# gebegebegebe/onnx-transformer

Hardware: AMD Instinct MI355X
Metric: decoded tokens/sec IWSLT14 de-en int8 greedy (batch 32 over 1 GPU, 71 steps) (higher is better)
Workload: dtype int8; 1 GPU; cfg2: greedy decode, src<=64 padded to 72, max_len=72, 32 sentences length-sorted over 1 rank(s); global_batch=32, per_gpu_batch=32, seq_len=72, parallelism=sentence-shard x1

## Files before the change

onnx-transformer_amd/csrc/qtx_common.h:

```cpp
#pragma once
#include <hip/hip_runtime.h>
#include <stdint.h>

#include <type_traits>

#define QTX_WAVE 64

typedef int v4i __attribute__((ext_vector_type(4)));
typedef float v4f __attribute__((ext_vector_type(4)));
typedef int v16i __attribute__((ext_vector_type(16)));

#ifdef QTX_STAMPS
static __device__ unsigned long long* qtx_stamp_buf;
#define QTX_STAMP_SETTER(unit)                                                            \
  extern "C" int qtx_debug_set_stamps_##unit(void* buf) {                                 \
    return (int)hipMemcpyToSymbol(HIP_SYMBOL(qtx_stamp_buf), &buf, sizeof(buf));          \
  }
#define QTX_STAMP(slot)                                                                 \
  do {                                                                                    \
    if (threadIdx.x == 0 && qtx_stamp_buf)                                                \
      qtx_stamp_buf[(blockIdx.y * gridDim.x + blockIdx.x) * 16 + (slot)] =                \
          __builtin_amdgcn_s_memtime();                                                   \
  } while (0)
#define QTX_NOW() ((long long)__builtin_amdgcn_s_memtime())
// ... 38 lines not shown
  v = fmaxf(v, dpp<0x141>(v));
  v = fmaxf(v, dpp<0x140>(v));
  return fmaxf(fmaxf(lane_f(v, 0), lane_f(v, 16)), fmaxf(lane_f(v, 32), lane_f(v, 48)));
}

template <int R>
__device__ __forceinline__ void wave_sum_n(float (&v)[R]) {
#pragma unroll
  for (int j = 0; j < R; ++j) v[j] = v[j] + dpp<0xB1>(v[j]);
#pragma unroll
  for (int j = 0; j < R; ++j) v[j] = v[j] + dpp<0x4E>(v[j]);
#pragma unroll
  for (int j = 0; j < R; ++j) v[j] = v[j] + dpp<0x141>(v[j]);
#pragma unroll
  for (int j = 0; j < R; ++j) v[j] = v[j] + dpp<0x140>(v[j]);
#pragma unroll
  for (int j = 0; j < R; ++j) v[j] = (lane_f(v[j], 0) + lane_f(v[j], 16)) + (lane_f(v[j], 32) + lane_f(v[j], 48));
}
template <int R>
__device__ __forceinline__ void wave_max_n(float (&v)[R]) {
#pragma unroll
  for (int j = 0; j < R; ++j) v[j] = fmaxf(v[j], dpp<0xB1>(v[j]));
#pragma unroll
  for (int j = 0; j < R; ++j) v[j] = fmaxf(v[j], dpp<0x4E>(v[j]));
#pragma unroll
  for (int j = 0; j < R; ++j) v[j] = fmaxf(v[j], dpp<0x141>(v[j]));
#pragma unroll
  for (int j = 0; j < R; ++j) v[j] = fmaxf(v[j], dpp<0x140>(v[j]));
#pragma unroll
  for (int j = 0; j < R; ++j)
    v[j] = fmaxf(fmaxf(lane_f(v[j], 0), lane_f(v[j], 16)), fmaxf(lane_f(v[j], 32), lane_f(v[j], 48)));
}

__device__ __forceinline__ float row16_sum(float v) {
  v = v + dpp<0xB1>(v);
  v = v + dpp<0x4E>(v);
  v = v + dpp<0x141>(v);
  return v + dpp<0x140>(v);
}
__device__ __forceinline__ float row16_max(float v) {
  v = fmaxf(v, dpp<0xB1>(v));
  v = fmaxf(v, dpp<0x4E>(v));
  v = fmaxf(v, dpp<0x141>(v));
  return fmaxf(v, dpp<0x140>(v));
}

__device__ __forceinline__ int wave_min_i32(int v) {
  auto d = [](int x, auto ctrl) {
    return __builtin_amdgcn_update_dpp(0x7fffffff, x, decltype(ctrl)::value, 0xF, 0xF, false);
  };
  v = min(v, d(v, std::integral_constant<int, 0xB1>{}));
  v = min(v, d(v, std::integral_constant<int, 0x4E>{}));
  v = min(v, d(v, std::integral_constant<int, 0x141>{}));
  v = min(v, d(v, std::integral_constant<int, 0x140>{}));
  return min(min(__builtin_amdgcn_readlane(v, 0), __builtin_amdgcn_readlane(v, 16)),
             min(__builtin_amdgcn_readlane(v, 32), __builtin_amdgcn_readlane(v, 48)));
}
template <int CTRL>
__device__ __forceinline__ int dpp_i32(int v) {
  return __builtin_amdgcn_update_dpp(0, v, CTRL, 0xF, 0xF, true);
}
__device__ __forceinline__ int row16_min_i32(int v) {
  v = min(v, dpp_i32<0xB1>(v));
  v = min(v, dpp_i32<0x4E>(v));
  v = min(v, dpp_i32<0x141>(v));
  return min(v, dpp_i32<0x140>(v));
// ... 128 lines not shown
__device__ __forceinline__ bool divisor_ok(float b) {
  const uint32_t m = __float_as_uint(b) & 0x7fffffffu;
  return m - 0x30800001u < 0x4e800000u - 0x30800001u;
}

__device__ __forceinline__ float div_const(float a, float b) {
  const float y = 1.0f / b;
  if (__builtin_expect(__ballot(!div_ok(a)) == 0ull, 1)) return div_cr(a, b, y);
  return a / b;
}
template <int R>
__device__ __forceinline__ void div_const_n(float (&a)[R], float b) {
  const float y = 1.0f / b;
  bool bad = false;
#pragma unroll
  for (int j = 0; j < R; ++j) bad |= !div_ok(a[j]);
  if (__builtin_expect(__ballot(bad) == 0ull, 1)) {
#pragma unroll
    for (int j = 0; j < R; ++j) a[j] = div_cr(a[j], b, y);
  } else {
#pragma unroll
    for (int j = 0; j < R; ++j) a[j] = a[j] / b;
  }
}

__device__ __forceinline__ float div127(float c) {
  return fmaf(c, 0x1.020408p-7f, c * 0x1.020408p-35f);
}

__device__ __forceinline__ float quant_scale(float absmax, float qmax) {
  return div_const(fmaxf(absmax, 1e-5f), qmax);
}
__device__ __forceinline__ int quant_val(float x, float s) { return (int)rintf(x / s); }
__device__ __forceinline__ float scale127(float a) {
  const bool big = a >= 0x1p60f;
  const float q = div_cr(big ? a * 0x1p-64f : a, 127.0f, 1.0f / 127.0f);
  return a == __builtin_inff() ? a : (big ? q * 0x1p64f : q);
}
__device__ __forceinline__ float rcp_cr(float s) {
  const float y0 = __builtin_amdgcn_rcpf(s);
  const float y = fmaf(fmaf(-s, y0, 1.0f), y0, y0);
  return s == __builtin_inff() ? 0.0f : y;
}

__device__ __forceinline__ uint32_t pack4_i8(int a, int b, int c, int d) {
  return (uint32_t)(a & 0xff) | ((uint32_t)(b & 0xff) << 8) | ((uint32_t)(c & 0xff) << 16) |
         ((uint32_t)(d & 0xff) << 24);
}

__host__ __device__ __forceinline__ long kp_off(long r, long k, long K) {
  return (((r >> 1) * (K >> 6) + (k >> 6)) << 7) + ((r & 1) << 6) + (k & 63);
}

template <class T>
__device__ __forceinline__ const T& ld_at(const T* base, unsigned byte_off) {
  return *reinterpret_cast<const T*>(reinterpret_cast<const char*>(base) + byte_off);
}
template <class T>
__device__ __forceinline__ void st_at(T* base, unsigned byte_off, const T& v) {
  *reinterpret_cast<T*>(reinterpret_cast<char*>(base) + byte_off) = v;
}

__device__ __forceinline__ float rint_biased(float q) { return q + 12582912.0f; }
__device__ __forceinline__ uint32_t pack4_biased(float t0, float t1, float t2, float t3) {
  const uint32_t p01 = __builtin_amdgcn_perm(__float_as_uint(t1), __float_as_uint(t0), 0x0c0c0400u);
  const uint32_t p23 = __builtin_amdgcn_perm(__float_as_uint(t3), __float_as_uint(t2), 0x0c0c0400u);
// ... 7 lines not shown
}
template <bool RELU>
__device__ __forceinline__ uint32_t pack4_codes(float q0, float q1, float q2, float q3) {
  if constexpr (RELU) return pack4_relu_u8(q0, q1, q2, q3);
  else return pack4_biased(rint_biased(q0), rint_biased(q1), rint_biased(q2), rint_biased(q3));
}

template <int N>
__device__ __forceinline__ void quant_pack(const float* x, float s, uint32_t* out) {
  static_assert(N % 4 == 0, "groups of 4");
  constexpr float BIAS = 12582912.0f;
  const float inv = __builtin_amdgcn_rcpf(s);
  float t[N];
  float dm = 0.0f;
#pragma unroll
  for (int i = 0; i < N; ++i) {
    const float r = x[i] * inv;
    t[i] = r + BIAS;
    dm = fmaxf(dm, fabsf(r - (t[i] - BIAS)));
  }
  if (__builtin_expect(__ballot(dm > 0.5f - 0x1p-13f) != 0ull, 0)) {
#pragma unroll
    for (int i = 0; i < N; ++i) t[i] = x[i] / s + BIAS;
  }
#pragma unroll
  for (int i = 0; i < N / 4; ++i) out[i] = pack4_biased(t[4 * i], t[4 * i + 1], t[4 * i + 2], t[4 * i + 3]);
}
__device__ __forceinline__ int quant_one(float x, float s) {
  float r = x * __builtin_amdgcn_rcpf(s);
  const bool near = fabsf((r - floorf(r)) - 0.5f) < 0x1p-13f;
  if (__builtin_expect(__ballot(near) != 0ull, 0)) r = x / s;
  return (int)rintf(r);
}

template <class PSF, class VF>
__device__ __forceinline__ float pv_dec_chains(int Sk, PSF&& ps, VF&& v) {
  float c[4] = {0.0f, 0.0f, 0.0f, 0.0f};
  for (int g = 0; g < Sk; g += 16)
#pragma unroll
    for (int e = 0; e < 4; ++e)
#pragma unroll
      for (int q = 0; q < 4; ++q) {
        const int j = g + 4 * q + e;
        if (j < Sk) c[q] = fmaf(ps(j), v(j), c[q]);
      }
  return (c[0] + c[1]) + (c[2] + c[3]);
}

__device__ __forceinline__ unsigned abs_bits(float x) { return __float_as_uint(fabsf(x)); }

template <int R>
__device__ __forceinline__ void ln_rows512(float (&v)[R][2][4], const float (&ga)[2][4],
                                           const float (&gb)[2][4]) {
  float mean[R], den[R];
#pragma unroll
  for (int j = 0; j < R; ++j) {
    float s = v[j][0][0];
#pragma unroll
    for (int c = 0; c < 2; ++c)
#pragma unroll
      for (int e = 0; e < 4; ++e)
        if (c | e) s = s + v[j][c][e];
    mean[j] = s;
  }
  wave_sum_n<R>(mean);
#pragma unroll
// ... 50 lines not shown
#pragma unroll
      for (int c = 0; c < 2; ++c)
#pragma unroll
        for (int e = 0; e < 4; ++e) v[j][c][e] = div_cr(v[j][c][e], den[j], y) + gb[c][e];
    }
  } else {
#pragma unroll
    for (int j = 0; j < R; ++j)
#pragma unroll
      for (int c = 0; c < 2; ++c)
#pragma unroll
        for (int e = 0; e < 4; ++e) v[j][c][e] = v[j][c][e] / den[j] + gb[c][e];
  }
}

__device__ __forceinline__ void ln_params512(const float* a, const float* b, int lane,
                                             float (&ga)[2][4], float (&gb)[2][4]) {
#pragma unroll
  for (int c = 0; c < 2; ++c) {
    const float4 ta = *reinterpret_cast<const float4*>(a + 4 * (lane + 64 * c));
    const float4 tb = *reinterpret_cast<const float4*>(b + 4 * (lane + 64 * c));
    ga[c][0] = ta.x; ga[c][1] = ta.y; ga[c][2] = ta.z; ga[c][3] = ta.w;
    gb[c][0] = tb.x; gb[c][1] = tb.y; gb[c][2] = tb.z; gb[c][3] = tb.w;
  }
}
template <int R>
__device__ __forceinline__ void ln_rows512(float (&v)[R][2][4], const float* a, const float* b,
                                           int lane) {
  float ga[2][4], gb[2][4];
  ln_params512(a, b, lane, ga, gb);
  ln_rows512<R>(v, ga, gb);
}

template <int R>
__device__ __forceinline__ void quant_rows512(const float (&v)[R][2][4], uint32_t (&q)[R][2],
                                              float (&sc)[R]) {
#pragma unroll
  for (int j = 0; j < R; ++j) {
    sc[j] = 0.0f;
#pragma unroll
    for (int c = 0; c < 2; ++c)
#pragma unroll
      for (int e = 0; e < 4; ++e) sc[j] = fmaxf(sc[j], fabsf(v[j][c][e]));
  }
  wave_max_n<R>(sc);
#pragma unroll
  for (int j = 0; j < R; ++j) sc[j] = fmaxf(sc[j], 1e-5f);
  div_const_n<R>(sc, 127.0f);
  constexpr float BIAS = 12582912.0f;
  float t[R][8];
  float dm = 0.0f;
#pragma unroll
  for (int j = 0; j < R; ++j) {
    const float inv = __builtin_amdgcn_rcpf(sc[j]);
#pragma unroll
    for (int i = 0; i < 8; ++i) {
      const float r = v[j][i >> 2][i & 3] * inv;
      t[j][i] = r + BIAS;
      dm = fmaxf(dm, fabsf(r - (t[j][i] - BIAS)));
    }
  }
  if (__builtin_expect(__ballot(dm > 0.5f - 0x1p-13f) != 0ull, 0)) {
#pragma unroll
    for (int j = 0; j < R; ++j)
#pragma unroll
      for (int i = 0; i < 8; ++i) t[j][i] = v[j][i >> 2][i & 3] / sc[j] + BIAS;
  }
#pragma unroll
  for (int j = 0; j < R; ++j) {
    q[j][0] = pack4_biased(t[j][0], t[j][1], t[j][2], t[j][3]);
    q[j][1] = pack4_biased(t[j][4], t[j][5], t[j][6], t[j][7]);
  }
}

}
```

onnx-transformer_amd/csrc/qtx_decode.hip:

```cpp
#include <cstdlib>

#include "qtx_common.h"
#include "qtx_kernels.h"
#include "qtx_knobs.h"

QTX_STAMP_SETTER(decode)

namespace qtx {

__device__ __forceinline__ uint4 unpack_i4(uint2 h) {
  auto sext = [](uint32_t v) { return v | ((v & 0x08080808u) * 0x1Eu); };
  const uint32_t lo0 = sext(h.x & 0x0F0F0F0Fu), hi0 = sext((h.x >> 4) & 0x0F0F0F0Fu);
  const uint32_t lo1 = sext(h.y & 0x0F0F0F0Fu), hi1 = sext((h.y >> 4) & 0x0F0F0F0Fu);
  uint4 o;
  o.x = __builtin_amdgcn_perm(hi0, lo0, 0x05010400u);
  o.y = __builtin_amdgcn_perm(hi0, lo0, 0x07030602u);
  o.z = __builtin_amdgcn_perm(hi1, lo1, 0x05010400u);
  o.w = __builtin_amdgcn_perm(hi1, lo1, 0x07030602u);
  return o;
}

struct KaLead { uint64_t w[7]; };
#define QTX_KA_PARAMS uint64_t ka0, uint64_t ka1, uint64_t ka2, uint64_t ka3, uint64_t ka4, \
                      uint64_t ka5, uint64_t ka6
// ... 84 lines not shown
    }
    issue_rest();
    if (tid < BM) sas[tid] = (tid < RB && m0 + tid < g.M) ? g.sa[m0 + tid] : 0.0f;
#pragma unroll
    for (int j = 0; j < NLD; ++j) {
      const int idx = tid + 256 * j, r = idx / CPR;
      if (TOT % 256 == 0 || idx < TOT)
        *reinterpret_cast<uint4*>(As + r * LDA + 16 * (idx % CPR)) =
            (m0 + r < g.M) ? v[j] : make_uint4(0, 0, 0, 0);
    }
  } else if constexpr (AMODE == A_LN) {
    float v[RPW][2][4];
#pragma unroll
    for (int j = 0; j < RPW; ++j) {
      const int m = min(m0 + wave + 4 * j, g.M - 1);
#pragma unroll
      for (int c = 0; c < 2; ++c) {
        const float4 t = ld_at(reinterpret_cast<const float4*>(g.X), 4u * (unsigned)(m * (int)g.ldx + 4 * (lane + 64 * c)));
        v[j][c][0] = t.x; v[j][c][1] = t.y; v[j][c][2] = t.z; v[j][c][3] = t.w;
      }
    }
    float ga[2][4], gb[2][4];
    ln_params512(g.ln_a, g.ln_b, lane, ga, gb);
    issue_rest();
    uint32_t q[RPW][2];
    float sc[RPW];
#if defined(QTX_ABL) && (QTX_ABL & 2)
#pragma unroll
    for (int j = 0; j < RPW; ++j) {
      q[j][0] = __float_as_uint(v[j][0][0]); q[j][1] = __float_as_uint(v[j][1][0]); sc[j] = v[j][0][1];
    }
#else
    ln_rows512<RPW>(v, ga, gb);
    quant_rows512<RPW>(v, q, sc);
#endif
#pragma unroll
    for (int j = 0; j < RPW; ++j) {
      const int r = wave + 4 * j;
      const bool ok = m0 + r < g.M;
      uint32_t* dst = reinterpret_cast<uint32_t*>(As + r * LDA);
      dst[lane] = ok ? q[j][0] : 0u;
      dst[lane + 64] = ok ? q[j][1] : 0u;
      if (lane == 0) sas[r] = ok ? sc[j] : 0.0f;
    }
  } else {
    constexpr bool OWN = AMODE == A_F32R;
    constexpr int NC = K / 256, RBT = RPW < 4 ? RPW : 4;
#pragma unroll
    for (int j0 = 0; j0 < RPW; j0 += RBT) {
      float4 t[RBT][NC];
      float pm[RBT][2];
#pragma unroll
      for (int jb = 0; jb < RBT; ++jb) {
        const int m = min(m0 + wave + 4 * (j0 + jb), g.M - 1);
#pragma unroll
        for (int c = 0; c < NC; ++c)
          t[jb][c] = ld_at(reinterpret_cast<const float4*>(g.X), 4u * (unsigned)(m * (int)g.ldx + 4 * (lane + 64 * c)));
        if constexpr (!OWN)
#pragma unroll
          for (int u = 0; u < 2; ++u)
            pm[jb][u] = ld_at(g.pmax_in, 4u * (unsigned)(min(lane + 64 * u, g.pmax_n - 1) * g.M + m));
      }
      if (j0 == 0) issue_rest();
#pragma unroll
      for (int jb = 0; jb < RBT; ++jb) {
        const int r = wave + 4 * (j0 + jb);
        const bool ok = m0 + r < g.M;
        float lm;
        if constexpr (OWN) {
          lm = 0.0f;
#pragma unroll
          for (int c = 0; c < NC; ++c)
            lm = fmaxf(lm, fmaxf(fmaxf(fabsf(t[jb][c].x), fabsf(t[jb][c].y)),
                                 fmaxf(fabsf(t[jb][c].z), fabsf(t[jb][c].w))));
        } else {
          lm = fmaxf(pm[jb][0], pm[jb][1]);
        }
        const float sc = quant_scale(wave_max(lm), 127.0f);
        uint32_t* dst = reinterpret_cast<uint32_t*>(As + r * LDA);
        float tf[4 * NC];
#pragma unroll
        for (int c = 0; c < NC; ++c) {
          tf[4 * c] = t[jb][c].x; tf[4 * c + 1] = t[jb][c].y;
          tf[4 * c + 2] = t[jb][c].z; tf[4 * c + 3] = t[jb][c].w;
        }
        uint32_t qd[NC];
#if defined(QTX_ABL) && (QTX_ABL & 8)
#pragma unroll
        for (int c = 0; c < NC; ++c) qd[c] = __float_as_uint(tf[4 * c] * sc);
#else
        quant_pack<4 * NC>(tf, sc, qd);
#endif
#pragma unroll
        for (int c = 0; c < NC; ++c) dst[lane + 64 * c] = ok ? qd[c] : 0u;
        if (lane == 0) sas[r] = ok ? sc : 0.0f;
      }
    }
  }
}

template <int MF, int RB, int K, int WBITS, int AMODE, int FLAGS>
__global__ __launch_bounds__(256) void k_skinny(QTX_KA_PARAMS, SkTail kt) {
  const SkinnyArgs g = sk_args<AMODE>(QTX_KA_VALS, kt);
  constexpr int BM = 16 * MF;
  static_assert(RB % 4 == 0 && RB <= BM, "rows per block");
  constexpr int KW = K / 4;
  constexpr int NS = KW / 64;
  constexpr int LDA = K + 16;
  __shared__ __attribute__((aligned(16))) uint8_t As[BM * LDA];
  __shared__ float sas[BM];
  __shared__ v4i red[4][MF][64];
// ... 72 lines not shown
  const int e = wave;
#pragma unroll
  for (int i = 0; i < MF; ++i) {
    {
      int sum = 0;
#pragma unroll
      for (int w = 0; w < 4; ++w) sum += reinterpret_cast<const int*>(&red[w][i][lane])[e];
      const int r = 16 * i + 4 * fg + e, row = m0 + r;
      const bool ok = cok && r < RB && row < g.M;
      float y = ((float)sum * sas[r]) * swc + bc;
      if constexpr (relu) y = y > 0.0f ? y : 0.0f;
      if constexpr (resid) y = rv[i] + y;
      if (ok) st_at(g.out, 4u * (unsigned)(row * (int)g.ldo + col), y);
      if constexpr (rmax) {
        float am = ok ? fabsf(y) : 0.0f;
        am = fmaxf(am, dpp<0xB1>(am));
        am = fmaxf(am, dpp<0x4E>(am));
        am = fmaxf(am, dpp<0x141>(am));
        am = fmaxf(am, dpp<0x140>(am));
        if (fr == 0 && r < RB && row < g.M) g.pmax_out[(long)blockIdx.x * g.M + row] = am;
      }
    }
  }
  QTX_STAMP(3);
}

template <bool OWN>
__global__ __launch_bounds__(512) void k_skinny8_ffn2(QTX_KA_PARAMS, SkTail kt) {
  const SkinnyArgs g = sk_args<OWN ? A_F32R : A_F32Q>(QTX_KA_VALS, kt);
  constexpr int K = 2048, RB = 4, KW = K / 8, NS = KW / 64, LDA = K + 16;
  __shared__ __attribute__((aligned(16))) uint8_t As[16 * LDA];
  __shared__ float sas[16];
  __shared__ v4i red[8][64];
  __shared__ float hmax[8];
  const int tid = threadIdx.x, wave = tid >> 6, lane = tid & 63;
  const int fr = lane & 15, fg = lane >> 4;
  const int n0 = blockIdx.x * 16, m0 = blockIdx.y * RB;
  const int r = wave >> 1, half = wave & 1;
  const int m = min(m0 + r, g.M - 1);
  float4 t[4];
#pragma unroll
  for (int c = 0; c < 4; ++c)
    t[c] = ld_at(reinterpret_cast<const float4*>(g.X), 4u * (unsigned)(m * (int)g.ldx + 4 * (lane + 64 * (4 * half + c))));
  float pm[2] = {0.0f, 0.0f};
  if constexpr (!OWN)
#pragma unroll
    for (int u = 0; u < 2; ++u) pm[u] = ld_at(g.pmax_in, 4u * (unsigned)(min(lane + 64 * u, g.pmax_n - 1) * g.M + m));
  const int n = min(n0 + fr, g.N - 1);
  uint4 wf[NS];
#pragma unroll
  for (int s = 0; s < NS; ++s)
    wf[s] = ld_at(reinterpret_cast<const uint4*>(g.W), (unsigned)(n * (int)g.ldw + wave * KW + 64 * s + 16 * fg));
  const int col = n0 + fr, cc = min(col, g.N - 1);
  const bool cok = col < g.N;
  const float swc = ld_at(g.sw, 4u * cc);
  __builtin_amdgcn_sched_barrier(0);
  const float rv = ld_at(g.res, 4u * (unsigned)(min(m0 + fg, g.M - 1) * (int)g.ldr + cc));
  const float bc = ld_at(g.bias, 4u * cc);
  {
    const bool ok = m0 + r < g.M;
    float rmax;
    if constexpr (OWN) {
      float lm = 0.0f;
#pragma unroll
      for (int c = 0; c < 4; ++c)
        lm = fmaxf(lm, fmaxf(fmaxf(fabsf(t[c].x), fabsf(t[c].y)), fmaxf(fabsf(t[c].z), fabsf(t[c].w))));
      lm = wave_max(lm);
      if (lane == 0) hmax[wave] = lm;
      __syncthreads();
      rmax = fmaxf(hmax[2 * r], hmax[2 * r + 1]);
    } else {
      rmax = wave_max(fmaxf(pm[0], pm[1]));
    }
    const float sc = quant_scale(rmax, 127.0f);
    float tf[16];
#pragma unroll
    for (int c = 0; c < 4; ++c) {
      tf[4 * c] = t[c].x; tf[4 * c + 1] = t[c].y; tf[4 * c + 2] = t[c].z; tf[4 * c + 3] = t[c].w;
    }
    uint32_t qd[4];
    quant_pack<16>(tf, sc, qd);
    uint32_t* dst = reinterpret_cast<uint32_t*>(As + r * LDA);
#pragma unroll
    for (int c = 0; c < 4; ++c) dst[lane + 64 * (4 * half + c)] = ok ? qd[c] : 0u;
    if (lane == 0 && half == 0) sas[r] = ok ? sc : 0.0f;
  }
  __syncthreads();
  v4i acc = v4i{0, 0, 0, 0};
#pragma unroll
  for (int s = 0; s < NS; ++s) {
    const v4i afr = *reinterpret_cast<const v4i*>(As + fr * LDA + wave * KW + 64 * s + 16 * fg);
    acc = __builtin_amdgcn_mfma_i32_16x16x64_i8(afr, __builtin_bit_cast(v4i, wf[s]), acc, 0, 0, 0);
  }
  red[wave][lane] = acc;
  __syncthreads();
  if (wave != 0) return;
  {
    const int e = fg, src = fr;
    int sum = 0;
#pragma unroll
    for (int w = 0; w < 8; ++w) sum += reinterpret_cast<const int*>(&red[w][src])[e];
    const int row = m0 + e;
    const float y = ((float)sum * sas[e]) * swc + bc;
    if (cok && row < g.M) st_at(g.out, 4u * (unsigned)(row * (int)g.ldo + col), rv + y);
  }
}

// ... 234 lines not shown
constexpr int DEC_MAXK = 128;

template <bool KV_NEW> struct DaLead;
template <> struct DaLead<true> {
  uint64_t y; int ldy, kv_bs; uint64_t kc, vc, skc, svc; int host_step1, zero;
};
template <> struct DaLead<false> {
  uint64_t y; int ldy, kv_bs; uint64_t kc, vc, skc, svc; int S, zero;
};
struct DaTail { const int* step; const uint8_t* mask; float* ctx; float* pmax; int B; };

template <bool KV_NEW> KaLead da_lead(const DecAttnArgs& a) {
  DaLead<KV_NEW> l{};
  l.y = ka_int(a.y); l.ldy = (int)a.ldy; l.kv_bs = (int)a.kv_bs;
  l.kc = ka_int(a.kc); l.vc = ka_int(a.vc); l.skc = ka_int(a.skc); l.svc = ka_int(a.svc);
  if constexpr (KV_NEW) l.host_step1 = a.host_step1; else l.S = a.S;
  return ka_pack(l);
}
template <bool KV_NEW>
__device__ __forceinline__ DecAttnArgs da_args(const KaLead& k, const DaTail& t) {
  const DaLead<KV_NEW> l = __builtin_bit_cast(DaLead<KV_NEW>, k);
  DecAttnArgs a{};
  a.y = ka_ptr<const float>(l.y); a.ldy = l.ldy; a.kv_bs = l.kv_bs;
  a.kc = ka_ptr<int8_t>(l.kc); a.vc = ka_ptr<int8_t>(l.vc);
  a.skc = ka_ptr<float>(l.skc); a.svc = ka_ptr<float>(l.svc);
  if constexpr (KV_NEW) a.host_step1 = l.host_step1; else a.S = l.S;
  a.step = t.step; a.mask = t.mask; a.ctx = t.ctx; a.pmax = t.pmax; a.B = t.B;
  return a;
}

template <bool KV_NEW, int NIT>
__global__ __launch_bounds__(64) void k_dec_attn(QTX_KA_PARAMS, DaTail kt) {
  const DecAttnArgs a = da_args<KV_NEW>(QTX_KA_VALS, kt);
  __shared__ __attribute__((aligned(16))) uint8_t Vs[DEC_MAXK * 64];
  __shared__ __attribute__((aligned(16))) float PS[DEC_MAXK];
  __shared__ __attribute__((aligned(16))) int8_t qs[KV_NEW ? 128 : 64];
  const int b = blockIdx.x, h = blockIdx.y, lane = threadIdx.x;
  const int fr = lane & 15, fg = lane >> 4;
  QTX_STAMP(0);
  const float* yr = a.y + (long)b * a.ldy;

  float4 yq[2], yk[2], yv[2];
#pragma unroll
  for (int c = 0; c < 2; ++c) {
    yq[c] = *reinterpret_cast<const float4*>(yr + 4 * (lane + 64 * c));
    if constexpr (KV_NEW) {
      yk[c] = *reinterpret_cast<const float4*>(yr + 512 + 4 * (lane + 64 * c));
      yv[c] = *reinterpret_cast<const float4*>(yr + 1024 + 4 * (lane + 64 * c));
    }
  }
  const float q_own = yr[h * 64 + lane];
  const float k_own = KV_NEW ? yr[512 + h * 64 + lane] : 0.0f;
  const float v_own = KV_NEW ? yr[1024 + h * 64 + lane] : 0.0f;
  __builtin_amdgcn_sched_barrier(0);
  const int nrows = KV_NEW ? (a.host_step1 > 0 ? a.host_step1 : (int)a.kv_bs) : a.S;
  const long kvb = (long)b * a.kv_bs;
  const long vgb = (long)b * ((a.kv_bs + 3) >> 2);
  const int vg = lane >> 4, vd = 4 * (lane & 15), glast = (nrows - 1) >> 2;
  const int8_t* const kbase = a.kc + kvb * 512 + h * 64;
  const int8_t* const vbase = a.vc + vgb * 2048 + h * 256;
  uint4 kr[NIT], vr[NIT];
#pragma unroll
  for (int i = 0; i < NIT; ++i) {
    const unsigned koff = (unsigned)(min(16 * i + fr, nrows - 1) * 512 + 16 * fg);
    const unsigned voff = (unsigned)(min(4 * i + vg, glast) * 2048 + 4 * vd);
    kr[i] = __builtin_bit_cast(uint4, __builtin_nontemporal_load(reinterpret_cast<const v4i*>(kbase + koff)));
    vr[i] = __builtin_bit_cast(uint4, __builtin_nontemporal_load(reinterpret_cast<const v4i*>(vbase + voff)));
  }
  const int j0 = min(lane, nrows - 1), j1 = min(lane + 64, nrows - 1);
  const float* const skb = a.skc + kvb;
  const float* const svb = a.svc + kvb;
  float sk0 = skb[(unsigned)j0], sk1 = skb[(unsigned)j1];
  float sv0 = svb[(unsigned)j0], sv1 = svb[(unsigned)j1];
  bool keep0 = true, keep1 = true;
  if constexpr (!KV_NEW) {
    const uint8_t* const mb = a.mask + (long)b * a.S;
    keep0 = mb[(unsigned)j0] != 0;
    keep1 = mb[(unsigned)j1] != 0;
  }
  const int step = !KV_NEW ? 0 : a.host_step1 > 0 ? a.host_step1 - 1 : min(max(*a.step, 0), (int)a.kv_bs - 1);
  int Sk = KV_NEW ? step + 1 : a.S;
  if constexpr (!KV_NEW) {
    const int last = wave_max_i32(max(keep0 && lane < a.S ? lane + 1 : 0,
                                      NIT > 4 && keep1 && lane + 64 < a.S ? lane + 65 : 0));
    if (last > 0) Sk = last;
  }

  auto amax8 = [](const float4 (&v)[2]) {
    float m = 0.0f;
#pragma unroll
    for (int c = 0; c < 2; ++c)
      m = fmaxf(m, fmaxf(fmaxf(fabsf(v[c].x), fabsf(v[c].y)), fmaxf(fabsf(v[c].z), fabsf(v[c].w))));
    return wave_max(m);
  };
  const float sq = quant_scale(amax8(yq), 127.0f);
  qs[lane] = (int8_t)quant_one(q_own, sq);
  int8_t kq = 0, vq = 0;
  float sk = 0.0f, sv = 0.0f;
  if constexpr (KV_NEW) {
    sk = quant_scale(amax8(yk), 127.0f);
    sv = quant_scale(amax8(yv), 127.0f);
    kq = (int8_t)quant_one(k_own, sk);
    vq = (int8_t)quant_one(v_own, sv);
    const long row = kvb + step;
    a.kc[row * 512 + h * 64 + lane] = kq;
    a.vc[((vgb + (step >> 2)) * 512 + h * 64 + lane) * 4 + (step & 3)] = vq;
    if (h == 0 && lane == 0) { a.skc[row] = sk; a.svc[row] = sv; }
    qs[64 + lane] = kq;
    if (lane == step) { sk0 = sk; sv0 = sv; }
    if (lane + 64 == step) { sk1 = sk; sv1 = sv; }
  }

  __syncthreads();
  const v4i qf = *reinterpret_cast<const v4i*>(qs + 16 * fg);
  if constexpr (KV_NEW) {
    const uint4 kn = *reinterpret_cast<const uint4*>(qs + 64 + 16 * fg);
    const bool own = fr == (step & 15);
#pragma unroll
    for (int i = 0; i < NIT; ++i)
      if (i == (step >> 4) && own) kr[i] = kn;
  }
  QTX_STAMP(1);

  v4i sacc[NIT];
#pragma unroll
  for (int i = 0; i < NIT; ++i)
    sacc[i] = __builtin_amdgcn_mfma_i32_16x16x64_i8(qf, __builtin_bit_cast(v4i, kr[i]), v4i{0, 0, 0, 0}, 0, 0, 0);
#pragma unroll
  for (int i = 0; i < NIT; ++i)
    *reinterpret_cast<uint4*>(Vs + (min(4 * i + vg, glast) * 64 + vd) * 4) = vr[i];
  if constexpr (KV_NEW) {
    Vs[((step >> 2) * 64 + lane) * 4 + (step & 3)] = (uint8_t)vq;
  }
  constexpr int NU = NIT > 4 ? 2 : 1;
  int dot[NU];
#pragma unroll
  for (int u = 0; u < NU; ++u) {
    dot[u] = sacc[4 * u][0];
#pragma unroll
    for (int t = 1; t < 4; ++t)
      if (4 * u + t < NIT) dot[u] = fg == t ? sacc[4 * u + t][0] : dot[u];
  }
  float sc[NU];
  bool live[NU];
  float lmax = -3.0e38f;
#pragma unroll
  for (int u = 0; u < NU; ++u) {
    live[u] = lane + 64 * u < Sk;
    const int acc = dot[u];
    float s = (((float)acc * sq) * (u ? sk1 : sk0)) * 0.125f;
    if (!(u ? keep1 : keep0)) s = -1.0e9f;
    sc[u] = s;
    lmax = live[u] ? fmaxf(lmax, s) : lmax;
  }
  const float m = wave_max(lmax);
  float lsum = 0.0f;
#pragma unroll
  for (int u = 0; u < NU; ++u) {
    const float e = qexp(sc[u] - m);
    sc[u] = e;
    lsum = lsum + (live[u] ? e : 0.0f);
  }
  const float den = wave_sum(lsum);
  const float rden = 1.0f / den;
  const int nk16 = (Sk + 15) & ~15;
#pragma unroll
  for (int u = 0; u < NU; ++u) {
    const int j = lane + 64 * u;
    const float ps = div127(rintf(div_cr(sc[u], den, rden) * 127.0f)) * (u ? sv1 : sv0);
    if (j < nk16) PS[j] = live[u] ? ps : 0.0f;
  }
  __syncthreads();
  QTX_STAMP(2);

  float c0 = 0.0f, c1 = 0.0f, c2 = 0.0f, c3 = 0.0f;
  const uint32_t* vl = reinterpret_cast<const uint32_t*>(Vs) + lane;
  float4 pg[NIT][4];
  uint32_t vg4[NIT][4];
#pragma unroll
  for (int g = 0; g < NIT; ++g) {
#pragma unroll
    for (int q = 0; q < 4; ++q) {
      pg[g][q] = *reinterpret_cast<const float4*>(PS + 16 * g + 4 * q);
      vg4[g][q] = vl[(4 * g + q) * 64];
    }
    __builtin_amdgcn_sched_barrier(0);
  }
  auto fmac = [](float& c, float p, float x) { asm("v_fmac_f32 %0, %1, %2" : "+v"(c) : "v"(p), "v"(x)); };
#pragma unroll
  for (int g = 0; g < NIT; ++g) {
    if (g == 0 || 16 * g < nk16) {
      float v[16];
#pragma unroll
      for (int q = 0; q < 4; ++q)
#pragma unroll
        for (int e = 0; e < 4; ++e) v[4 * q + e] = (float)(int8_t)(vg4[g][q] >> (8 * e));
      const float4 p0 = pg[g][0], p1 = pg[g][1], p2 = pg[g][2], p3 = pg[g][3];
      fmac(c0, p0.x, v[0]);  fmac(c1, p1.x, v[4]);  fmac(c2, p2.x, v[8]);  fmac(c3, p3.x, v[12]);
      fmac(c0, p0.y, v[1]);  fmac(c1, p1.y, v[5]);  fmac(c2, p2.y, v[9]);  fmac(c3, p3.y, v[13]);
      fmac(c0, p0.z, v[2]);  fmac(c1, p1.z, v[6]);  fmac(c2, p2.z, v[10]); fmac(c3, p3.z, v[14]);
      fmac(c0, p0.w, v[3]);  fmac(c1, p1.w, v[7]);  fmac(c2, p2.w, v[11]); fmac(c3, p3.w, v[15]);
    }
  }
  const float acc = (c0 + c1) + (c2 + c3);
  QTX_STAMP(3);

  st_at(a.ctx, 4u * (unsigned)(b * 512 + h * 64 + lane), acc);
  if (a.pmax) {
    const float am = wave_max(fabsf(acc));
    if (lane == 0) a.pmax[(long)h * a.B + b] = am;
  }
  QTX_STAMP(4);
}

template <bool KV_NEW>
hipError_t dec_attn_nit(const DecAttnArgs& a, int B, int nrows, hipStream_t st) {
  const dim3 grid(B, 8), block(64);
// ... 35 lines not shown
  const long bg = i >> 9;
  const int g = (int)(bg % G4), b = (int)(bg / G4);
  const int8_t* src = v + (long)blockIdx.y * v_ls;
  uint32_t w = 0;
#pragma unroll
  for (int e = 0; e < 4; ++e) {
    const int j = 4 * g + e;
    const uint32_t byte = j < S ? (uint8_t)src[((long)b * S + j) * 512 + d] : 0u;
    w |= byte << (8 * e);
  }
  reinterpret_cast<uint32_t*>(out + (long)blockIdx.y * o_ls)[i] = w;
}

hipError_t launch_vgroup4(const int8_t* v, long v_ls, int L, int B, int S, int8_t* out,
                          long o_ls, hipStream_t st) {
  if (B <= 0 || S <= 0 || L <= 0) return hipSuccess;
  const long n = (long)B * ((S + 3) / 4) * 512;
  k_vgroup4<<<dim3((unsigned)((n + 255) / 256), L), dim3(256), 0, st>>>(v, v_ls, B, S, out, o_ls);
  return hipGetLastError();
}

__global__ __launch_bounds__(256) void k_quant_h2048(const float* X, long ldx, int M,
                                                     int8_t* q, float* s) {
  __shared__ float wm[4];
  const int m = blockIdx.x, tid = threadIdx.x, wave = tid >> 6, lane = tid & 63;
  const float* xr = X + (long)m * ldx + 512 * wave;
  float4 t[2];
#pragma unroll
  for (int c = 0; c < 2; ++c) t[c] = *reinterpret_cast<const float4*>(xr + 4 * (lane + 64 * c));
  float lm = 0.0f;
#pragma unroll
  for (int c = 0; c < 2; ++c)
    lm = fmaxf(lm, fmaxf(fmaxf(fabsf(t[c].x), fabsf(t[c].y)), fmaxf(fabsf(t[c].z), fabsf(t[c].w))));
  lm = wave_max(lm);
  if (lane == 0) wm[wave] = lm;
  __syncthreads();
  const float sc = quant_scale(fmaxf(fmaxf(wm[0], wm[1]), fmaxf(wm[2], wm[3])), 127.0f);
  float tf[8];
#pragma unroll
  for (int c = 0; c < 2; ++c) {
    tf[4 * c] = t[c].x; tf[4 * c + 1] = t[c].y; tf[4 * c + 2] = t[c].z; tf[4 * c + 3] = t[c].w;
  }
  uint32_t qd[2];
  quant_pack<8>(tf, sc, qd);
  uint32_t* dst = reinterpret_cast<uint32_t*>(q + (long)m * 2048 + 512 * wave);
#pragma unroll
  for (int c = 0; c < 2; ++c) dst[lane + 64 * c] = qd[c];
  if (tid == 0) s[m] = sc;
}

hipError_t launch_quant_h2048(const float* X, long ldx, int M, int8_t* q, float* s,
                              hipStream_t st) {
  if (M <= 0) return hipSuccess;
  k_quant_h2048<<<dim3(M), dim3(256), 0, st>>>(X, ldx, M, q, s);
  return hipGetLastError();
}

constexpr int GEN_Q = 32;

template <bool REC>
__global__ __launch_bounds__(1024) void k_generator_mfma(const float* Wm, int V, int M,
                                                         const float* bias, const float* x,
                                                         long ldx, const float* ln_a,
                                                         const float* ln_b, float* logits,
                                                         float* rec) {
  __shared__ __attribute__((aligned(16))) float X[16][514];
  __shared__ __attribute__((aligned(16))) v4f part[3][4][64];
// ... 378 lines not shown
      id = 0;
    } else if (!(w.m2 > w.m1 - ARG_DELTA) && w.i1 != 0x7fffffff) {
      id = w.i1;
    } else {
      id = tok_exact(kt.logits + (long)m * V, V, w.m1, lane);
    }
    ids[j] = max(min(id, V - 1), 0);
  }
  float4 em[RPW][2];
#pragma unroll
  for (int j = 0; j < RPW; ++j)
#pragma unroll
    for (int c = 0; c < 2; ++c)
      em[j][c] = ld_at(ka_ptr<const float4>(l.lut), 16u * (unsigned)(ids[j] * 128 + lane + 64 * c));
#pragma unroll
  for (int j = 0; j < RPW; ++j) {
    const int r = wave + 4 * j, m = min(m0 + r, M - 1);
    const float sc = 0x1.6a09e6p+4f;
    const bool st = blockIdx.x == 0 && m0 + r < M;
#pragma unroll
    for (int c = 0; c < 2; ++c) {
      const float4 e = em[j][c];
      const float4 x = make_float4(e.x * sc + pe[c].x, e.y * sc + pe[c].y, e.z * sc + pe[c].z,
                                   e.w * sc + pe[c].w);
      v[j][c][0] = x.x; v[j][c][1] = x.y; v[j][c][2] = x.z; v[j][c][3] = x.w;
      if (st) st_at(reinterpret_cast<float4*>(kt.xres), 16u * (unsigned)(m * 128 + lane + 64 * c), x);
    }
    if (st && lane == 0 && kt.pos < kt.ids_bs) kt.ids[m * kt.ids_bs + kt.pos] = ids[j];
  }
  {
    uint32_t q[RPW][2];
    float sc[RPW];
    ln_rows512<RPW>(v, ga, gb);
    quant_rows512<RPW>(v, q, sc);
#pragma unroll
    for (int j = 0; j < RPW; ++j) {
      const int r = wave + 4 * j;
      const bool ok = m0 + r < M;
      uint32_t* dst = reinterpret_cast<uint32_t*>(As + r * LDA);
      dst[lane] = ok ? q[j][0] : 0u;
      dst[lane + 64] = ok ? q[j][1] : 0u;
      if (lane == 0) sas[r] = ok ? sc[j] : 0.0f;
    }
  }
  __syncthreads();
  v4i acc = v4i{0, 0, 0, 0};
#pragma unroll
  for (int s = 0; s < NS; ++s) {
    const v4i afr = *reinterpret_cast<const v4i*>(As + fr * LDA + 64 * s + 16 * fg);
    acc = __builtin_amdgcn_mfma_i32_16x16x64_i8(afr, __builtin_bit_cast(v4i, wf[s]), acc, 0, 0, 0);
  }
  if (fg < RPW) tail[wave][16 * fg + fr] = acc;
  __builtin_amdgcn_wave_barrier();
#pragma unroll
  for (int j = 0; j < RPW; ++j) {
    const int vv = reinterpret_cast<const int*>(&tail[wave][16 * j + fr])[fg];
    const int r = fg + 4 * j, row = m0 + r;
    const float y = ((float)vv * sas[r]) * swc + bc;
    if (row < M) st_at(kt.out, 4u * (unsigned)(row * kt.ldo + col), y);
  }
}

hipError_t launch_skinny_tok(const SkinnyArgs& g, const TokArgs& t, hipStream_t st) {
  if (g.M <= 0) return hipSuccess;
  const long lim = 1L << 30;
  if (g.K != 512 || g.N % 64 || g.flags || g.ldw != 512 || t.V < 1 || t.V > ARG_MAXV ||
      t.pos < 1 || (long)g.M * t.V >= lim || (long)g.M * g.ldo >= lim || (long)g.N * g.ldw >= lim)
// ... 498 lines not shown
```

Baseline: 200,700 tokens/s.

## Load V groups straight to registers and use integer-bit absmax reductions

In decode attention, V is now loaded from global memory straight into per-lane registers, and the new step's value is patched in place. This replaces staging V through a shared-memory tile. The absmax reductions for quantization scales now do unsigned-integer max on the float bits, using DPP with bound_ctrl and an integer floor. They also use a cheaper divide-by-127 with a single range check. The OWN quant GEMM path now loads the other half-row so each wave computes the full row max itself, removing a shared-memory exchange and a __syncthreads. The change trims LDS traffic, barriers and float-max latency, at the cost of more VGPRs and more global loads.

```diff
diff --git a/onnx-transformer_amd/csrc/qtx_common.h b/onnx-transformer_amd/csrc/qtx_common.h
--- a/onnx-transformer_amd/csrc/qtx_common.h
+++ b/onnx-transformer_amd/csrc/qtx_common.h
@@ -94,6 +94,41 @@
     v[j] = fmaxf(fmaxf(lane_f(v[j], 0), lane_f(v[j], 16)), fmaxf(lane_f(v[j], 32), lane_f(v[j], 48)));
 }
 
+template <int CTRL>
+__device__ __forceinline__ uint32_t dpp_u32(uint32_t v) {
+  return (uint32_t)__builtin_amdgcn_update_dpp(0, (int)v, CTRL, 0xF, 0xF, true);
+}
+__device__ __forceinline__ uint32_t lane_u32(uint32_t v, int l) {
+  return (uint32_t)__builtin_amdgcn_readlane((int)v, l);
+}
+__device__ __forceinline__ float wave_absmax(float f, float floor = 0.0f) {
+  uint32_t v = __float_as_uint(f);
+  v = max(v, dpp_u32<0xB1>(v));
+  v = max(v, dpp_u32<0x4E>(v));
+  v = max(v, dpp_u32<0x141>(v));
+  v = max(v, dpp_u32<0x140>(v));
+  return __uint_as_float(max(max(max(lane_u32(v, 0), lane_u32(v, 16)), max(lane_u32(v, 32), lane_u32(v, 48))),
+                             __float_as_uint(floor)));
+}
+template <int R>
+__device__ __forceinline__ void wave_absmax_n(float (&f)[R], float floor = 0.0f) {
+  uint32_t v[R];
+#pragma unroll
+  for (int j = 0; j < R; ++j) v[j] = __float_as_uint(f[j]);
+#pragma unroll
+  for (int j = 0; j < R; ++j) v[j] = max(v[j], dpp_u32<0xB1>(v[j]));
+#pragma unroll
+  for (int j = 0; j < R; ++j) v[j] = max(v[j], dpp_u32<0x4E>(v[j]));
+#pragma unroll
+  for (int j = 0; j < R; ++j) v[j] = max(v[j], dpp_u32<0x141>(v[j]));
+#pragma unroll
+  for (int j = 0; j < R; ++j) v[j] = max(v[j], dpp_u32<0x140>(v[j]));
+#pragma unroll
+  for (int j = 0; j < R; ++j)
+    f[j] = __uint_as_float(max(max(max(lane_u32(v[j], 0), lane_u32(v[j], 16)), max(lane_u32(v[j], 32), lane_u32(v[j], 48))),
+                               __float_as_uint(floor)));
+}
+
 __device__ __forceinline__ float row16_sum(float v) {
   v = v + dpp<0xB1>(v);
   v = v + dpp<0x4E>(v);
@@ -288,6 +323,23 @@
   return div_const(fmaxf(absmax, 1e-5f), qmax);
 }
 __device__ __forceinline__ int quant_val(float x, float s) { return (int)rintf(x / s); }
+__device__ __forceinline__ float absmax_scale127(float a) {
+  if (__builtin_expect(__float_as_uint(a) < 0x5d800000u, 1)) return div_cr(a, 127.0f, 1.0f / 127.0f);
+  return a / 127.0f;
+}
+template <int R>
+__device__ __forceinline__ void absmax_scale127_n(float (&a)[R]) {
+  uint32_t mx = 0u;
+#pragma unroll
+  for (int j = 0; j < R; ++j) mx = max(mx, __float_as_uint(a[j]));
+  if (__builtin_expect(mx < 0x5d800000u, 1)) {
+#pragma unroll
+    for (int j = 0; j < R; ++j) a[j] = div_cr(a[j], 127.0f, 1.0f / 127.0f);
+  } else {
+#pragma unroll
+    for (int j = 0; j < R; ++j) a[j] = a[j] / 127.0f;
+  }
+}
 __device__ __forceinline__ float scale127(float a) {
   const bool big = a >= 0x1p60f;
   const float q = div_cr(big ? a * 0x1p-64f : a, 127.0f, 1.0f / 127.0f);
@@ -361,6 +413,22 @@
   if (__builtin_expect(__ballot(near) != 0ull, 0)) r = x / s;
   return (int)rintf(r);
 }
+template <int R>
+__device__ __forceinline__ void quant_one_n(const float (&x)[R], const float (&s)[R], int (&q)[R]) {
+  float r[R];
+  bool near = false;
+#pragma unroll
+  for (int j = 0; j < R; ++j) {
+    r[j] = x[j] * __builtin_amdgcn_rcpf(s[j]);
+    near |= fabsf((r[j] - floorf(r[j])) - 0.5f) < 0x1p-13f;
+  }
+  if (__builtin_expect(__ballot(near) != 0ull, 0)) {
+#pragma unroll
+    for (int j = 0; j < R; ++j) r[j] = x[j] / s[j];
+  }
+#pragma unroll
+  for (int j = 0; j < R; ++j) q[j] = (int)rintf(r[j]);
+}
 
 template <class PSF, class VF>
 __device__ __forceinline__ float pv_dec_chains(int Sk, PSF&& ps, VF&& v) {
@@ -477,7 +545,7 @@
   ln_rows512<R>(v, ga, gb);
 }
 
-template <int R>
+template <int R, bool IMAX = false>
 __device__ __forceinline__ void quant_rows512(const float (&v)[R][2][4], uint32_t (&q)[R][2],
                                               float (&sc)[R]) {
 #pragma unroll
@@ -488,10 +556,15 @@
 #pragma unroll
       for (int e = 0; e < 4; ++e) sc[j] = fmaxf(sc[j], fabsf(v[j][c][e]));
   }
-  wave_max_n<R>(sc);
-#pragma unroll
-  for (int j = 0; j < R; ++j) sc[j] = fmaxf(sc[j], 1e-5f);
-  div_const_n<R>(sc, 127.0f);
+  if constexpr (IMAX) {
+    wave_absmax_n<R>(sc, 1e-5f);
+    absmax_scale127_n<R>(sc);
+  } else {
+    wave_max_n<R>(sc);
+#pragma unroll
+    for (int j = 0; j < R; ++j) sc[j] = fmaxf(sc[j], 1e-5f);
+    div_const_n<R>(sc, 127.0f);
+  }
   constexpr float BIAS = 12582912.0f;
   float t[R][8];
   float dm = 0.0f;
diff --git a/onnx-transformer_amd/csrc/qtx_decode.hip b/onnx-transformer_amd/csrc/qtx_decode.hip
--- a/onnx-transformer_amd/csrc/qtx_decode.hip
+++ b/onnx-transformer_amd/csrc/qtx_decode.hip
@@ -140,7 +140,7 @@
     }
 #else
     ln_rows512<RPW>(v, ga, gb);
-    quant_rows512<RPW>(v, q, sc);
+    quant_rows512<RPW, true>(v, q, sc);
 #endif
 #pragma unroll
     for (int j = 0; j < RPW; ++j) {
@@ -184,7 +184,9 @@
         } else {
           lm = fmaxf(pm[jb][0], pm[jb][1]);
         }
-        const float sc = quant_scale(wave_max(lm), 127.0f);
+        float sc;
+        if constexpr (OWN) sc = absmax_scale127(wave_absmax(lm, 1e-5f));
+        else sc = quant_scale(wave_max(lm), 127.0f);
         uint32_t* dst = reinterpret_cast<uint32_t*>(As + r * LDA);
         float tf[4 * NC];
 #pragma unroll
@@ -323,7 +325,6 @@
   __shared__ __attribute__((aligned(16))) uint8_t As[16 * LDA];
   __shared__ float sas[16];
   __shared__ v4i red[8][64];
-  __shared__ float hmax[8];
   const int tid = threadIdx.x, wave = tid >> 6, lane = tid & 63;
   const int fr = lane & 15, fg = lane >> 4;
   const int n0 = blockIdx.x * 16, m0 = blockIdx.y * RB;
@@ -334,9 +335,15 @@
   for (int c = 0; c < 4; ++c)
     t[c] = ld_at(reinterpret_cast<const float4*>(g.X), 4u * (unsigned)(m * (int)g.ldx + 4 * (lane + 64 * (4 * half + c))));
   float pm[2] = {0.0f, 0.0f};
-  if constexpr (!OWN)
+  float4 to[4] = {};
+  if constexpr (!OWN) {
 #pragma unroll
     for (int u = 0; u < 2; ++u) pm[u] = ld_at(g.pmax_in, 4u * (unsigned)(min(lane + 64 * u, g.pmax_n - 1) * g.M + m));
+  } else {
+#pragma unroll
+    for (int c = 0; c < 4; ++c)
+      to[c] = ld_at(reinterpret_cast<const float4*>(g.X), 4u * (unsigned)(m * (int)g.ldx + 4 * (lane + 64 * (4 * (half ^ 1) + c))));
+  }
   const int n = min(n0 + fr, g.N - 1);
   uint4 wf[NS];
 #pragma unroll
@@ -350,20 +357,18 @@
   const float bc = ld_at(g.bias, 4u * cc);
   {
     const bool ok = m0 + r < g.M;
-    float rmax;
+    float sc;
     if constexpr (OWN) {
       float lm = 0.0f;
 #pragma unroll
-      for (int c = 0; c < 4; ++c)
+      for (int c = 0; c < 4; ++c) {
         lm = fmaxf(lm, fmaxf(fmaxf(fabsf(t[c].x), fabsf(t[c].y)), fmaxf(fabsf(t[c].z), fabsf(t[c].w))));
-      lm = wave_max(lm);
-      if (lane == 0) hmax[wave] = lm;
-      __syncthreads();
-      rmax = fmaxf(hmax[2 * r], hmax[2 * r + 1]);
+        lm = fmaxf(lm, fmaxf(fmaxf(fabsf(to[c].x), fabsf(to[c].y)), fmaxf(fabsf(to[c].z), fabsf(to[c].w))));
+      }
+      sc = absmax_scale127(wave_absmax(lm, 1e-5f));
     } else {
-      rmax = wave_max(fmaxf(pm[0], pm[1]));
-    }
-    const float sc = quant_scale(rmax, 127.0f);
+      sc = quant_scale(wave_max(fmaxf(pm[0], pm[1])), 127.0f);
+    }
     float tf[16];
 #pragma unroll
     for (int c = 0; c < 4; ++c) {
@@ -664,7 +669,6 @@
 template <bool KV_NEW, int NIT>
 __global__ __launch_bounds__(64) void k_dec_attn(QTX_KA_PARAMS, DaTail kt) {
   const DecAttnArgs a = da_args<KV_NEW>(QTX_KA_VALS, kt);
-  __shared__ __attribute__((aligned(16))) uint8_t Vs[DEC_MAXK * 64];
   __shared__ __attribute__((aligned(16))) float PS[DEC_MAXK];
   __shared__ __attribute__((aligned(16))) int8_t qs[KV_NEW ? 128 : 64];
   const int b = blockIdx.x, h = blockIdx.y, lane = threadIdx.x;
@@ -688,16 +692,14 @@
   const int nrows = KV_NEW ? (a.host_step1 > 0 ? a.host_step1 : (int)a.kv_bs) : a.S;
   const long kvb = (long)b * a.kv_bs;
   const long vgb = (long)b * ((a.kv_bs + 3) >> 2);
-  const int vg = lane >> 4, vd = 4 * (lane & 15), glast = (nrows - 1) >> 2;
+  const int glast = (nrows - 1) >> 2;
   const int8_t* const kbase = a.kc + kvb * 512 + h * 64;
   const int8_t* const vbase = a.vc + vgb * 2048 + h * 256;
-  uint4 kr[NIT], vr[NIT];
+  uint4 kr[NIT];
 #pragma unroll
   for (int i = 0; i < NIT; ++i) {
     const unsigned koff = (unsigned)(min(16 * i + fr, nrows - 1) * 512 + 16 * fg);
-    const unsigned voff = (unsigned)(min(4 * i + vg, glast) * 2048 + 4 * vd);
     kr[i] = __builtin_bit_cast(uint4, __builtin_nontemporal_load(reinterpret_cast<const v4i*>(kbase + koff)));
-    vr[i] = __builtin_bit_cast(uint4, __builtin_nontemporal_load(reinterpret_cast<const v4i*>(vbase + voff)));
   }
   const int j0 = min(lane, nrows - 1), j1 = min(lane + 64, nrows - 1);
   const float* const skb = a.skc + kvb;
@@ -710,6 +712,16 @@
     keep0 = mb[(unsigned)j0] != 0;
     keep1 = mb[(unsigned)j1] != 0;
   }
+  uint32_t vg4[NIT][4];
+  __builtin_amdgcn_sched_barrier(0);
+#pragma unroll
+  for (int g = 0; g < NIT; ++g)
+#pragma unroll
+    for (int q = 0; q < 4; ++q) {
+      const int grp = g < NIT - 1 ? min(4 * g, max(glast - 3, 0)) + q : min(4 * g + q, glast);
+      vg4[g][q] = __builtin_nontemporal_load(
+          reinterpret_cast<const uint32_t*>(vbase + (unsigned)(grp * 2048 + 4 * lane)));
+    }
   const int step = !KV_NEW ? 0 : a.host_step1 > 0 ? a.host_step1 - 1 : min(max(*a.step, 0), (int)a.kv_bs - 1);
   int Sk = KV_NEW ? step + 1 : a.S;
   if constexpr (!KV_NEW) {
@@ -718,22 +730,32 @@
     if (last > 0) Sk = last;
   }
 
-  auto amax8 = [](const float4 (&v)[2]) {
+  auto lmax8 = [](const float4 (&v)[2]) {
     float m = 0.0f;
 #pragma unroll
     for (int c = 0; c < 2; ++c)
       m = fmaxf(m, fmaxf(fmaxf(fabsf(v[c].x), fabsf(v[c].y)), fmaxf(fabsf(v[c].z), fabsf(v[c].w))));
-    return wave_max(m);
+    return m;
   };
-  const float sq = quant_scale(amax8(yq), 127.0f);
-  qs[lane] = (int8_t)quant_one(q_own, sq);
+  float sq;
   int8_t kq = 0, vq = 0;
   float sk = 0.0f, sv = 0.0f;
   if constexpr (KV_NEW) {
-    sk = quant_scale(amax8(yk), 127.0f);
-    sv = quant_scale(amax8(yv), 127.0f);
-    kq = (int8_t)quant_one(k_own, sk);
-    vq = (int8_t)quant_one(v_own, sv);
+    float am[3] = {lmax8(yq), lmax8(yk), lmax8(yv)};
+    wave_absmax_n<3>(am, 1e-5f);
+    absmax_scale127_n<3>(am);
+    const float own[3] = {q_own, k_own, v_own};
+    int code[3];
+    quant_one_n<3>(own, am, code);
+    sq = am[0]; sk = am[1]; sv = am[2];
+    qs[lane] = (int8_t)code[0];
+    kq = (int8_t)code[1];
+    vq = (int8_t)code[2];
+  } else {
+    sq = absmax_scale127(wave_absmax(lmax8(yq), 1e-5f));
+    qs[lane] = (int8_t)quant_one(q_own, sq);
+  }
+  if constexpr (KV_NEW) {
     const long row = kvb + step;
     a.kc[row * 512 + h * 64 + lane] = kq;
     a.vc[((vgb + (step >> 2)) * 512 + h * 64 + lane) * 4 + (step & 3)] = vq;
@@ -758,12 +780,6 @@
 #pragma unroll
   for (int i = 0; i < NIT; ++i)
     sacc[i] = __builtin_amdgcn_mfma_i32_16x16x64_i8(qf, __builtin_bit_cast(v4i, kr[i]), v4i{0, 0, 0, 0}, 0, 0, 0);
-#pragma unroll
-  for (int i = 0; i < NIT; ++i)
-    *reinterpret_cast<uint4*>(Vs + (min(4 * i + vg, glast) * 64 + vd) * 4) = vr[i];
-  if constexpr (KV_NEW) {
-    Vs[((step >> 2) * 64 + lane) * 4 + (step & 3)] = (uint8_t)vq;
-  }
   constexpr int NU = NIT > 4 ? 2 : 1;
   int dot[NU];
 #pragma unroll
@@ -806,15 +822,26 @@
   QTX_STAMP(2);
 
   float c0 = 0.0f, c1 = 0.0f, c2 = 0.0f, c3 = 0.0f;
-  const uint32_t* vl = reinterpret_cast<const uint32_t*>(Vs) + lane;
+  if constexpr (KV_NEW) {
+    const int pq = (step >> 2) & 3, sh = 8 * (step & 3);
+    const uint32_t ins = (uint32_t)(uint8_t)vq << sh, keep = ~(0xffu << sh);
+    auto patch = [&](uint32_t (&f)[4], bool here) {
+#pragma unroll
+      for (int q = 0; q < 4; ++q) f[q] = here && q == pq ? (f[q] & keep) | ins : f[q];
+    };
+    if (a.host_step1 > 0) {
+      patch(vg4[NIT - 1], true);
+    } else {
+#pragma unroll
+      for (int g = 0; g < NIT; ++g) patch(vg4[g], g == (step >> 4));
+    }
+  }
   float4 pg[NIT][4];
-  uint32_t vg4[NIT][4];
 #pragma unroll
   for (int g = 0; g < NIT; ++g) {
 #pragma unroll
     for (int q = 0; q < 4; ++q) {
       pg[g][q] = *reinterpret_cast<const float4*>(PS + 16 * g + 4 * q);
-      vg4[g][q] = vl[(4 * g + q) * 64];
     }
     __builtin_amdgcn_sched_barrier(0);
   }
@@ -916,7 +943,7 @@
 #pragma unroll
   for (int c = 0; c < 2; ++c)
     lm = fmaxf(lm, fmaxf(fmaxf(fabsf(t[c].x), fabsf(t[c].y)), fmaxf(fabsf(t[c].z), fabsf(t[c].w))));
-  lm = wave_max(lm);
+  lm = wave_absmax(lm);
   if (lane == 0) wm[wave] = lm;
   __syncthreads();
   const float sc = quant_scale(fmaxf(fmaxf(wm[0], wm[1]), fmaxf(wm[2], wm[3])), 127.0f);
@@ -1361,7 +1388,7 @@
     uint32_t q[RPW][2];
     float sc[RPW];
     ln_rows512<RPW>(v, ga, gb);
-    quant_rows512<RPW>(v, q, sc);
+    quant_rows512<RPW, true>(v, q, sc);
 #pragma unroll
     for (int j = 0; j < RPW; ++j) {
       const int r = wave + 4 * j;
```

Result: faster. 202,900 tokens/s (median of 6 runs) (+1.1%).
